# AI-sandbox/gnomix

Measured on AMD Instinct MI355X. Metric: haplotypes/sec (+ windows/sec) chr22 7-ancestry inference, higher is better.
Workload: dtype int8 x 7-digit fixed-point weights -> exact i32/i64 logits, f64 sigmoid (logistic base); f32 (tree smoother)

## Files before the change

gnomix_amd/_lib.py:

```python
from __future__ import annotations

import atexit
import ctypes as C
import os
import weakref

_HERE = os.path.dirname(os.path.abspath(__file__))
SO_PATH = os.environ.get("GNX_LIBRARY") or os.path.join(_HERE, "libgnomix_hip.so")

GNX_ABI_VERSION = 16
GNX_OK, GNX_EINVAL, GNX_ENOMEM, GNX_EHIP, GNX_EUNSUPPORTED, GNX_ESTATE, GNX_ESTALE = 0, -1, -2, -3, -4, -5, -6
BASE_NONE, BASE_LOGISTIC, BASE_COVRSK_SVC, BASE_FOREST, BASE_RFOREST, BASE_KNN, BASE_NB, BASE_LDA = 0, 1, 2, 3, 4, 5, 6, 7
SVC_KERNEL_SUBSTRINGS, SVC_KERNEL_POLY, SVC_KERNEL_ALL_LENGTHS, SVC_KERNEL_RBF = 0, 1, 2, 3
SMOOTH_NONE, SMOOTH_XGB, SMOOTH_CRF, SMOOTH_CNN = 0, 1, 2, 3
K_BASE_LOGISTIC, K_SMOOTH_XGB, K_BASE_COVRSK, K_SMOOTH_CRF, K_GNOFIX, K_SMOOTH_ROWS, K_CALIBRATE, K_BASE_FOREST, K_SMOOTH_CNN = range(9)
KERNEL_NAMES = {K_BASE_LOGISTIC: "k_base_logistic", K_SMOOTH_XGB: "k_smooth_xgb", K_BASE_COVRSK: "k_base_covrsk",
                K_SMOOTH_CRF: "k_smooth_crf", K_GNOFIX: "k_gnofix", K_SMOOTH_ROWS: "k_smooth_rows", K_CALIBRATE: "k_calibrate",
                K_BASE_FOREST: "k_base_forest", K_SMOOTH_CNN: "k_smooth_cnn"}


class GnxLibraryError(ImportError):
    pass


# ... 133 lines not shown
    "gnx_init": (C.c_int, [C.c_int, C.POINTER(_VP)]),
    "gnx_ctx_free": (None, [_VP]),
    "gnx_last_error": (C.c_char_p, [_VP]),
    "gnx_set_stream": (C.c_int, [_VP, _VP]),
    "gnx_reset_stream": (C.c_int, [_VP]),
    "gnx_synchronize": (C.c_int, [_VP]),
    "gnx_model_load": (C.c_int, [_VP, C.POINTER(ModelDesc), C.POINTER(_VP)]),
    "gnx_model_load_nb": (C.c_int, [_VP, C.POINTER(ModelDesc), C.POINTER(NbWindow), C.POINTER(_VP)]),
    "gnx_model_load_lda": (C.c_int, [_VP, C.POINTER(ModelDesc), C.POINTER(LdaWindow), C.POINTER(_VP)]),
    "gnx_model_free": (None, [_VP]),
    "gnx_model_get_info": (C.c_int, [_VP, C.POINTER(ModelInfo)]),
    "gnx_model_set_calibrate": (C.c_int, [_VP, _I]),
    "gnx_model_export_prepared": (C.c_int, [_VP, _VP, _I64, C.POINTER(_I64)]),
    "gnx_base_predict": (C.c_int, [_VP, _VP, _I64, _I64, _VP, _VP]),
    "gnx_base_predict_dev": (C.c_int, [_VP, _VP, _I64, _I64, _VP, _VP]),
    "gnx_smooth_predict": (C.c_int, [_VP, _VP, _I, _I64, _VP, _VP, _VP]),
    "gnx_smooth_predict_dev": (C.c_int, [_VP, _VP, _I, _I64, _VP, _VP, _VP]),
    "gnx_infer": (C.c_int, [_VP, _VP, _I64, _I64, _VP, _VP, _VP]),
    "gnx_infer_dev": (C.c_int, [_VP, _VP, _I64, _I64, _VP, _VP, _VP]),
    "gnx_packed_row_bytes": (_I64, [_I64]),
    "gnx_pack_x": (C.c_int, [_VP, _I64, _I64, _I64, _VP, _I64, _I]),
    "gnx_unpack_x_dev": (C.c_int, [_VP, _VP, _I64, _I64, _I64, _VP, _I64]),
    "gnx_infer_packed": (C.c_int, [_VP, _VP, _I64, _I64, _VP, _VP, _VP]),
    "gnx_infer_packed_dev": (C.c_int, [_VP, _VP, _I64, _I64, _VP, _VP, _VP]),
    "gnx_base_predict_packed_dev": (C.c_int, [_VP, _VP, _I64, _I64, _VP, _VP]),
    "gnx_smooth_rows": (C.c_int, [_VP, _VP, _I64, _VP]),
    "gnx_calibrate_rows": (C.c_int, [_VP, _VP, _I, _I64, _VP]),
    "gnx_gnofix": (C.c_int, [_VP, _VP, _I64, _VP, _I64, C.c_int32, _VP, _VP]),
    "gnx_gnofix_dev": (C.c_int, [_VP, _VP, _I64, _VP, _I64, C.c_int32, _VP, _VP]),
    "gnx_gnofix_packed_dev": (C.c_int, [_VP, _VP, _I64, _VP, _I64, C.c_int32, _VP, _VP]),
# ... 208 lines not shown
```

gnomix_amd/csrc/gnx_api.hip:

```cpp
#include <algorithm>
#include <cmath>
#include <cstdio>
#include <cstdlib>
#include <cstring>
#include <limits>
#include <new>
#include <thread>
#include <utility>

#include "gnx_internal.h"

int gnx_fail(gnx_ctx* ctx, int code, const std::string& msg) {
  if (ctx) ctx->err = msg;
  return code;
}
static inline int fail(gnx_ctx* ctx, int code, const std::string& msg) { return gnx_fail(ctx, code, msg); }

#define HIPCHK(ctx, expr)                                                                      \
  do {                                                                                         \
    hipError_t e__ = (expr);                                                                   \
    if (e__ != hipSuccess)                                                                     \
      return fail((ctx), GNX_EHIP, std::string(#expr) + ": " + hipGetErrorString(e__));        \
  } while (0)

// ... 80 lines not shown
  if (const char* e = std::getenv("GNX_SM_TUNE")) std::sscanf(e, "%d,%d", &t.smf_rpl, &t.smf_nw);
  if (const char* e = std::getenv("GNX_CRF_FLAGS")) t.crf_flags = atoi(e);
  if (const char* e = std::getenv("GNX_LDS_PAD")) std::sscanf(e, "%d,%d", &t.lr_lds_pad, &t.sm_lds_pad);
  if (const char* e = std::getenv("GNX_CRF_IMPL")) t.crf_impl = !std::strcmp(e, "scan") ? 1 : !std::strcmp(e, "row") ? 2 : !std::strcmp(e, "lanes") ? 3 : !std::strcmp(e, "quad") ? 4 : !std::strcmp(e, "mm") ? 5 : 0;
  t.forest_threads = geti("GNX_FOREST_T", 0);
  t.forest_wrun = geti("GNX_FOREST_WRUN", 0);
  t.forest_halves = geti("GNX_FOREST_H", 0);
  t.forest_flags = geti("GNX_FOREST_FLAGS", 0);
  t.forest_impl = geti("GNX_FOREST_IMPL", 0);
  if (const char* e = std::getenv("GNX_HOST_BATCH")) t.host_batch = std::atoll(e);
  t.h2d_overlap = geti("GNX_H2D_OVERLAP", 1);
  t.debug = std::getenv("GNX_DEBUG") ? atoi(std::getenv("GNX_DEBUG")) : 0;
  if (const char* e = std::getenv("GNX_GNOFIX_IMPL")) t.gnofix_impl = std::string(e) == "f32" ? 1 : 0;
  t.gnofix_threads = geti("GNX_GNOFIX_T", 0);
  t.gnofix_aux = geti("GNX_GNOFIX_AUX", 1);
}

extern "C" {

int gnx_abi_version(void) { return GNX_ABI_VERSION; }

int gnx_build_flags(void) {
#ifdef GNX_EXPERIMENTS
  return GNX_BUILD_EXPERIMENTS;
#else
  return 0;
#endif
}

static void want_hw_queues() { setenv("GPU_MAX_HW_QUEUES", "8", 0); }
// ... 270 lines not shown
  if (!m) return;
  gnx_ctx unbound;
  if (!m->ctx) (void)hipGetDevice(&unbound.device);
  gnx_device_scope bind(m->ctx ? m->ctx : &unbound);
  if (m->ctx && m->ctx->usable) (void)hipStreamSynchronize(m->ctx->stream);
  for (void* p : m->dev_allocs) (void)hipFree(p);
  delete m;
}

int gnx_model_get_info(const gnx_model* m, gnx_model_info* out) {
  if (!m || !out) return GNX_EINVAL;
  *out = m->info;
  return GNX_OK;
}

int gnx_base_predict_dev(gnx_model* m, const int8_t* dX, int64_t N, int64_t ldx, float* d_b32, double* d_b64) {
  if (!m) return GNX_EINVAL;
  gnx_ctx* ctx = m->ctx;
  if (N < 0 || ldx < m->info.C || (N > 0 && !dX)) return fail(ctx, GNX_EINVAL, "base_predict: bad X / N / ldx");
  if (N == 0 || (!d_b32 && !d_b64)) return GNX_OK;
  GNX_BIND_DEVICE(ctx);
  if (m->info.base_kind == GNX_BASE_KNN) return gnx_base_predict_knn(m, dX, N, ldx, d_b32, d_b64);
  if (m->info.base_kind == GNX_BASE_NB) return gnx_base_predict_nb(m, dX, N, ldx, d_b32, d_b64);
  if (m->info.base_kind == GNX_BASE_LDA) return gnx_base_predict_lda(m, dX, N, ldx, d_b32, d_b64);
  if (m->info.base_kind == GNX_BASE_COVRSK_SVC && m->rbf) {
    ProfScope ps(ctx, GNX_K_BASE_COVRSK);
    return gnx_base_predict_rbf(m, dX, N, ldx, d_b32, d_b64);
  }
  if (m->info.base_kind == GNX_BASE_COVRSK_SVC) {
    const int64_t Cp = m->info.C + 2 * m->info.ctx, nwp = (Cp + 31) / 32 + 2;
    int rc = ws_reserve(ctx, ctx->ws_bits, (size_t)N * 2 * nwp * 4);
    if (rc != GNX_OK) return rc;
    ProfScope ps(ctx, GNX_K_BASE_COVRSK);
    HIPCHK(ctx, gnx_launch_pack_bits(dX, N, ldx, m->info.C, m->info.ctx, nwp, (uint32_t*)ctx->ws_bits.p, ctx->stream));
    CovRSKLaunch L{};
// ... 48 lines not shown
    const size_t need = (size_t)m->info.C + 128;
    if (ctx->ws_lastrow.cap < need) {
      int rc = ws_reserve(ctx, ctx->ws_lastrow, need);
      if (rc != GNX_OK) return rc;
      HIPCHK(ctx, hipMemsetAsync(ctx->ws_lastrow.p, 0, ctx->ws_lastrow.cap, ctx->stream));
    }
    HIPCHK(ctx, hipMemcpyAsync(ctx->ws_lastrow.p, dX + (N - 1) * ldx, (size_t)m->info.C, hipMemcpyDeviceToDevice, ctx->stream));
  }
  BaseLRLaunch L{};
  L.X = dX;
  L.last_row = (const int8_t*)ctx->ws_lastrow.p;
  L.N = N; L.ldx = ldx; L.d = m->lr;
  L.h_win_chunk0 = m->lr_h_win_chunk0.data(); L.h_win_chunk1 = m->lr_h_win_chunk1.data();
  L.W = (int32_t)m->info.W; L.A = m->info.A;
  L.b32 = d_b32; L.b64 = d_b64;
  ProfScope ps(ctx, GNX_K_BASE_LOGISTIC);
  if (m->lr_i8) {
    const bool dl = ctx->tune.lr_dl < 0 ? m->lr.NT >= 2 : ctx->tune.lr_dl != 0;
    hipError_t e = hipErrorNotSupported;
#ifdef GNX_EXPERIMENTS
    if (ctx->tune.lr_ws) e = gnx_launch_base_logistic_i8_ws(L, ctx->n_cu, ctx->tune, ctx->stream);
    if (e == hipErrorNotSupported && ctx->tune.lr_w512) e = gnx_launch_base_logistic_i8_w512(L, ctx->n_cu, ctx->tune, ctx->stream);
    if (e == hipErrorNotSupported && ctx->tune.lr_flat > 0 && m->lr.V8F) e = gnx_launch_base_logistic_i8_fl(L, ctx->n_cu, ctx->tune, ctx->stream);
#endif
    if (e == hipErrorNotSupported && dl) e = gnx_launch_base_logistic_i8_dl(L, ctx->n_cu, ctx->tune, ctx->stream);
    if (e == hipErrorNotSupported) e = gnx_launch_base_logistic_i8(L, ctx->n_cu, ctx->tune, ctx->stream);
    HIPCHK(ctx, e);
  }
  else HIPCHK(ctx, gnx_launch_base_logistic(L, ctx->n_cu, ctx->stream));
  return GNX_OK;
}

static int smooth_raw_dev(gnx_model* m, const void* dB, int b_is_f64, int64_t N, float* d_p32, double* d_p64, int32_t* d_lab);

int gnx_smooth_predict_dev(gnx_model* m, const void* dB, int b_is_f64, int64_t N, float* d_p32, double* d_p64,
                           int32_t* d_lab) {
  if (!m) return GNX_EINVAL;
  gnx_ctx* ctx = m->ctx;
  GNX_BIND_DEVICE(ctx);
  if (!(m->calibrate_on && m->calib_off)) return smooth_raw_dev(m, dB, b_is_f64, N, d_p32, d_p64, d_lab);
  if (N < 0 || (N > 0 && !dB)) return fail(ctx, GNX_EINVAL, "smooth_predict: bad B / N");
  if (N == 0) return GNX_OK;
  const size_t n = (size_t)N * m->info.W * m->info.A;
  const bool nat64 = m->info.smooth_kind == GNX_SMOOTH_CRF;
  int rc = ws_reserve(ctx, ctx->ws_cal, n * (nat64 ? 8 : 4));
  if (rc != GNX_OK) return rc;
  rc = smooth_raw_dev(m, dB, b_is_f64, N, nat64 ? nullptr : (float*)ctx->ws_cal.p, nat64 ? (double*)ctx->ws_cal.p : nullptr, nullptr);
  if (rc != GNX_OK) return rc;
  CalibLaunch L{};
  L.in = ctx->ws_cal.p; L.in_is_f64 = nat64; L.R = N * m->info.W; L.A = m->info.A;
  L.off = m->calib_off; L.x = m->calib_x; L.y = m->calib_y; L.thr_f32 = m->calib_f32;
  L.out64 = d_p64; L.out32 = d_p32; L.labels = d_lab;
  ProfScope ps(ctx, GNX_K_CALIBRATE);
  HIPCHK(ctx, gnx_launch_calibrate(L, ctx->stream));
  return GNX_OK;
}

static int smooth_raw_dev(gnx_model* m, const void* dB, int b_is_f64, int64_t N, float* d_p32, double* d_p64, int32_t* d_lab) {
  gnx_ctx* ctx = m->ctx;
  if (N < 0 || (N > 0 && !dB)) return fail(ctx, GNX_EINVAL, "smooth_predict: bad B / N");
  if (N == 0) return GNX_OK;
  if (m->info.smooth_kind == GNX_SMOOTH_XGB) {
    const size_t n = (size_t)N * m->info.W * m->info.A;
    if (!d_p32) {
      int rc = ws_reserve(ctx, ctx->ws_misc, n * sizeof(float));
      if (rc != GNX_OK) return rc;
      d_p32 = (float*)ctx->ws_misc.p;
    }
    SmoothXGBLaunch L{};
    L.B = dB; L.b_is_f64 = b_is_f64; L.N = N;
    L.W = (int32_t)m->info.W; L.A = m->info.A; L.S = m->info.S;
    L.d = m->xgb; L.proba = d_p32; L.proba64 = d_p64; L.labels = d_lab;
#ifdef GNX_EXPERIMENTS
    const bool h64 = m->xgb.rk_packed && m->xgb.impl == 2 && gnx_smooth_h64_waves(m->xgb, m->info.A, m->info.S) > 0;
    if (m->xgb.impl == 2 && !h64) return fail(ctx, GNX_EUNSUPPORTED, "GNX_SMOOTH_IMPL=h64: the model's strip does not fit the LDS");
#else
// ... 15 lines not shown
      if (rc != GNX_OK) return rc;
    }
#endif
    ProfScope ps(ctx, GNX_K_SMOOTH_XGB);
#ifdef GNX_EXPERIMENTS
    if (bs) {
      HIPCHK(ctx, gnx_launch_smooth_xgb_bs(L, (uint16_t*)ctx->ws_marg.p, ctx->n_cu, ctx->tune, ctx->stream));
      return GNX_OK;
    }
#endif
#ifdef GNX_EXPERIMENTS
    if (h64) HIPCHK(ctx, gnx_launch_smooth_xgb_h64(L, (uint16_t*)ctx->ws_rank.p, ctx->tune, ctx->stream));
    else
#endif
    if (m->xgb.rk_packed) {
      const bool h32 = (m->xgb.impl == 5 || (m->xgb.impl == 6 && (N + 31) / 32 * ((L.W + GNX_H32_WPB - 1) / GNX_H32_WPB) >= ctx->n_cu)) &&
                       gnx_smooth_h32_fits(m->xgb, L.A, L.S);
      if (h32) {
        HIPCHK(ctx, gnx_launch_smooth_xgb_h32(L, ctx->stream));
        return GNX_OK;
      }
      if (L.d.impl == 5 || L.d.impl == 6) L.d.impl = 3;
      HIPCHK(ctx, gnx_launch_smooth_xgb_rk(L, ctx->tune, ctx->stream));
    } else HIPCHK(ctx, gnx_launch_smooth_xgb(L, ctx->tune, ctx->stream));
    return GNX_OK;
  }
  if (m->info.smooth_kind == GNX_SMOOTH_CRF) {
    const size_t n = (size_t)N * m->info.W * m->info.A;
    int rc;
    if ((rc = ws_reserve(ctx, ctx->ws_misc, n * sizeof(double) + 4096)) != GNX_OK) return rc;
    double* alpha = (double*)ctx->ws_misc.p;
    if ((rc = ws_reserve(ctx, ctx->ws_scale, (size_t)2 * N * m->info.W * sizeof(double))) != GNX_OK) return rc;
    if ((rc = ws_reserve(ctx, ctx->ws_psi, n * sizeof(double) + 4096)) != GNX_OK) return rc;
// ... 57 lines not shown
  const char* in0 = reinterpret_cast<const char*>(dP);
  const bool in_xu = ctx->ws_xu.p && in0 >= (const char*)ctx->ws_xu.p && in0 < (const char*)ctx->ws_xu.p + ctx->ws_xu.cap;
  gnx_devbuf& wide = in_xu ? ctx->ws_xu2 : ctx->ws_xu;
  int rc = ws_reserve(ctx, wide, (size_t)N * ldx + 256);
  if (rc != GNX_OK) return rc;
  HIPCHK(ctx, gnx_launch_unpack2(dP, N, ldp, C, (int8_t*)wide.p, ldx, ctx->stream));
  return gnx_base_predict_dev(m, (const int8_t*)wide.p, N, ldx, d_b32, d_b64);
}

static int infer_any_dev(gnx_model* m, const void* dIn, bool packed, int64_t N, int64_t ld, float* d_p32, double* d_p64, int32_t* d_lab) {
  gnx_ctx* ctx = m->ctx;
  if (N <= 0) return N == 0 ? GNX_OK : fail(ctx, GNX_EINVAL, "infer: N < 0");
  GNX_BIND_DEVICE(ctx);
  const size_t n = (size_t)N * m->info.W * m->info.A;
  const bool f64 = (m->info.smooth_kind == GNX_SMOOTH_CRF);
  int rc = ws_reserve(ctx, f64 ? ctx->ws_b64 : ctx->ws_b32, n * (f64 ? 8 : 4));
  if (rc != GNX_OK) return rc;
  float* b32 = f64 ? nullptr : (float*)ctx->ws_b32.p;
  double* b64 = f64 ? (double*)ctx->ws_b64.p : nullptr;
  rc = packed ? gnx_base_predict_packed_dev(m, (const uint8_t*)dIn, N, ld, b32, b64) : gnx_base_predict_dev(m, (const int8_t*)dIn, N, ld, b32, b64);
  if (rc != GNX_OK) return rc;
  return gnx_smooth_predict_dev(m, f64 ? ctx->ws_b64.p : ctx->ws_b32.p, f64, N, d_p32, d_p64, d_lab);
}

int gnx_infer_dev(gnx_model* m, const int8_t* dX, int64_t N, int64_t ldx, float* d_p32, double* d_p64, int32_t* d_lab) {
  if (!m) return GNX_EINVAL;
  return infer_any_dev(m, dX, false, N, ldx, d_p32, d_p64, d_lab);
}

static int64_t hap_batch(const gnx_model* m, int64_t N, int64_t ldx) {
  int64_t nb = ((int64_t)1 << 30) / std::max<int64_t>(ldx, 1);
// ... 82 lines not shown
  int rc;
  if (nbuf == 2 && (rc = pipe_init(ctx)) != GNX_OK) return rc;
  const int64_t ldx_dev = packed ? ((C + 15) / 16) * 16 : ld;
  const size_t in_bytes = (((size_t)nb * ld + 64) + 255) & ~(size_t)255;
  gnx_devbuf& wsin = packed ? ctx->ws_pk : ctx->ws_x;
  if ((rc = ws_reserve(ctx, wsin, in_bytes * nbuf)) != GNX_OK) return rc;
  const bool p2 = packed && lr_p2_usable(m);
  if (packed && !p2 && (rc = ws_reserve(ctx, ctx->ws_xu, (size_t)nb * ldx_dev + 256)) != GNX_OK) return rc;
  const size_t p32_b = (nb * WA * 4 + 255) & ~(size_t)255, p64_b = (nb * WA * 8 + 255) & ~(size_t)255, lab_b = (nb * Wn * 4 + 255) & ~(size_t)255;
  if ((rc = ws_reserve(ctx, ctx->ws_p32, p32_b * nbuf)) != GNX_OK) return rc;
  if (p64 && (rc = ws_reserve(ctx, ctx->ws_p64, p64_b * nbuf)) != GNX_OK) return rc;
  if (lab && (rc = ws_reserve(ctx, ctx->ws_lab, lab_b * nbuf)) != GNX_OK) return rc;
  {
    const bool f64 = (m->info.smooth_kind == GNX_SMOOTH_CRF);
    if ((rc = ws_reserve(ctx, f64 ? ctx->ws_b64 : ctx->ws_b32, nb * WA * (f64 ? 8 : 4))) != GNX_OK) return rc;
  }
  hipStream_t sc = ctx->stream, si = nbuf == 2 ? ctx->s_in : ctx->stream, so = nbuf == 2 ? ctx->s_out : ctx->stream;
  const uint8_t* hsrc = (const uint8_t*)src;
  const int64_t n_batches = (N + nb - 1) / nb;
  auto issue_h2d = [&](int64_t i) -> int {
    const int b = (int)(i % nbuf);
    const int64_t n0 = i * nb, n = std::min(nb, N - n0);
    if (nbuf == 2 && i >= 2) HIPCHK(ctx, hipStreamWaitEvent(si, ctx->ev_done[b], 0));
    HIPCHK(ctx, hipMemcpyAsync((char*)wsin.p + (size_t)b * in_bytes, hsrc + (size_t)n0 * ld, (size_t)(n - 1) * ld + row_bytes,
                               hipMemcpyHostToDevice, si));
    if (nbuf == 2) HIPCHK(ctx, hipEventRecord(ctx->ev_in[b], si));
    return GNX_OK;
  };
  if ((rc = issue_h2d(0)) != GNX_OK) return rc;
  for (int64_t i = 0; i < n_batches; ++i) {
// ... 681 lines not shown
```

gnomix_amd/csrc/gnx_internal.h:

```cpp
#pragma once
#include <hip/hip_runtime.h>
#include <stdint.h>
#include <algorithm>
#include <memory>
#include <string>
#include <vector>

#include "../../include/gnomix_hip.h"
#include "gnx_rank_table.h"

struct gnx_devbuf {
  void* p = nullptr;
  size_t cap = 0;
};

struct gnx_prof_pair {
  hipEvent_t a, b;
  int kid;
};

struct gnx_tune {
  int lr_bpc = 0, lr_want = 0;
  int lr_mt = 0, lr_waves = 0;
  int lr_flags = 0;
// ... 9 lines not shown
  int sm_pair = 1;
  int smf_rpl = 0, smf_nw = 0;
  int crf_impl = 0;
  int crf_flags = 0;
  int forest_threads = 0;
  int forest_wrun = 0;
  int forest_halves = 0;
  int forest_impl = 0;
  int forest_flags = 0;
  int64_t host_batch = 0;
  int h2d_overlap = 1;
  int lr_lds_pad = 0, sm_lds_pad = 0;
  int gnofix_impl = 0;
  int gnofix_aux = 1;
  int gnofix_threads = 0;
  int debug = 0;
};

#define GNX_LDS_OPTIN(bytes, ...)                                                                                  \
  do {                                                                                                             \
    const hipError_t e_optin_ = hipFuncSetAttribute(reinterpret_cast<const void*>(&__VA_ARGS__),                   \
                                                    hipFuncAttributeMaxDynamicSharedMemorySize, (int)(bytes));     \
    if (e_optin_ != hipSuccess) return e_optin_;                                                                   \
  } while (0)

struct gnx_ctx {
  int device = 0;
  gnx_tune tune;
  hipStream_t stream = nullptr;
  bool own_stream = false;
// ... 51 lines not shown
  const int8_t* X;
  const int8_t* last_row;
  int64_t N, ldx;
  BaseLRDev d;
  const int32_t* h_win_chunk0;
  const int32_t* h_win_chunk1;
  int32_t W, A, wch;
  int32_t n_htiles;
  int32_t n_rg8;
  int32_t flags;
  int32_t max_chunks;
  int32_t max_wins;
  float* b32;
  double* b64;
  unsigned long long* dbg = nullptr;
};

struct SmoothXGBDev {
  const uint8_t* packed = nullptr;
  const int32_t* group_tree0 = nullptr;
  const int32_t* group_class = nullptr;
  int32_t n_groups = 0, n_trees = 0, D = 0, tree_bytes = 0, max_group = 0;
  float base_score = 0.5f;
  const uint8_t* rk_packed = nullptr;
  const float* rk_thr = nullptr;
  const GnxRankEntry* rk_lut = nullptr;
  const int32_t* rk_group_tree0 = nullptr;
  const int32_t* rk_group_class = nullptr;
  int32_t rk_K = 0, rk_steps = 0, rk_stride = 0, rk_tree_bytes = 0, rk_n_groups = 0, rk_max_group = 0;
  int32_t rk_bits = 0;
  int32_t rk_rpl = 0;
// ... 61 lines not shown
  __builtin_memcpy(&fv, row + n4.x, 4);
  return (fv < __uint_as_float(n4.y)) ? __uint_as_float(n4.z) : __uint_as_float(n4.w);
}
#endif

struct SmoothXGBLaunch {
  const void* B;
  int32_t b_is_f64;
  int64_t N;
  int32_t W, A, S;
  SmoothXGBDev d;
  float* proba;
  float* marg;
  double* proba64;
  int32_t* labels;
};


struct SmoothCRFLaunch {
  const void* B;
  int32_t b_is_f64;
  int64_t N;
  int32_t W, A;
  const double* state;
  const double* etrans;
  double* psi;
  double* alpha;
  double* scale;
  double* proba64;
  float* proba32;
// ... 219 lines not shown
  *out = (const T*)p;
  return GNX_OK;
}


hipError_t gnx_launch_gt2_to_x(const uint8_t* G, int64_t V, int64_t ldg, int64_t n0, int64_t N, const int32_t* src, int64_t C,
                               int8_t* X, int64_t ldx, hipStream_t s);
hipError_t gnx_launch_gt2_to_p2(const uint8_t* G, int64_t V, int64_t ldg, int64_t n0, int64_t N, const int32_t* src, int64_t C,
                                uint8_t* P, int64_t ldp, hipStream_t s);
hipError_t gnx_launch_p2_to_gt2(const uint8_t* P, int64_t N, int64_t ldp, int64_t n0, const int32_t* cols, int64_t V, uint8_t* G,
                                int64_t ldg, hipStream_t s);
hipError_t gnx_launch_x_to_gt2(const int8_t* X, int64_t N, int64_t ldx, int64_t n0, const int32_t* cols, int64_t V, uint8_t* G,
                               int64_t ldg, hipStream_t s);
hipError_t gnx_launch_base_logistic(const BaseLRLaunch& L, int n_cu, hipStream_t s);
hipError_t gnx_launch_base_logistic_i8(const BaseLRLaunch& L, int n_cu, const gnx_tune& tune, hipStream_t s);
hipError_t gnx_launch_base_logistic_i8_dl(const BaseLRLaunch& L, int n_cu, const gnx_tune& tune, hipStream_t s);
hipError_t gnx_launch_base_logistic_p2(const BaseLRLaunch& L, int n_cu, const gnx_tune& tune, hipStream_t s);
#ifdef GNX_EXPERIMENTS
hipError_t gnx_launch_base_logistic_i8_w512(const BaseLRLaunch& L, int n_cu, const gnx_tune& tune, hipStream_t s);
hipError_t gnx_launch_base_logistic_i8_ws(const BaseLRLaunch& L, int n_cu, const gnx_tune& tune, hipStream_t s);
hipError_t gnx_launch_base_logistic_i8_fl(const BaseLRLaunch& L, int n_cu, const gnx_tune& tune, hipStream_t s);
hipError_t gnx_launch_smooth_xgb_h64(const SmoothXGBLaunch& L, uint16_t* Rk, const gnx_tune& tune, hipStream_t s);
int gnx_smooth_h64_waves(const SmoothXGBDev& d, int A, int S);
size_t gnx_smooth_h64_rank_bytes(int64_t N, int W, int A, int S);
#endif
hipError_t gnx_launch_fb_len(const float* d_proba, int64_t N, int64_t W, int A, uint8_t* d_len, unsigned long long* d_line_len, hipStream_t s);
hipError_t gnx_launch_fb_emit(const float* d_proba, int64_t N, int64_t W, int A, const uint8_t* d_len, const char* d_pb, const int64_t* d_po,
                              const int64_t* d_line_off, char* d_body, hipStream_t s);
hipError_t gnx_launch_smooth_xgb(const SmoothXGBLaunch& L, const gnx_tune& tune, hipStream_t s);
hipError_t gnx_launch_smooth_xgb_rk(const SmoothXGBLaunch& L, const gnx_tune& tune, hipStream_t s);
// ... 45 lines not shown
```

gnomix_amd/csrc/k_base_logistic_i8.hip:

```cpp
#include <algorithm>
#include <cstdio>
#include <cstdlib>

#include "gnx_internal.h"
#include "gnx_exp.h"

namespace {

typedef int v4i __attribute__((ext_vector_type(4)));
struct __attribute__((packed, aligned(1))) xbytes16 { v4i v; };

constexpr int LIMBS = 7;

__device__ __forceinline__ v4i load_x16(const int8_t* p) {
  xbytes16 r;
  __builtin_memcpy(&r, p, 16);
  return r.v;
}

__device__ __forceinline__ double combine(const v4i (&acc)[LIMBS], int reg, double scale) {
  long long lo = (long long)acc[0][reg] + ((long long)acc[1][reg] << 8) + ((long long)acc[2][reg] << 16);
  long long hi = (long long)acc[3][reg] + ((long long)acc[4][reg] << 8) + ((long long)acc[5][reg] << 16) +
                 ((long long)acc[6][reg] << 24);
  return ((double)hi * 16777216.0 + (double)lo) * scale;
// ... 18 lines not shown
    const int last_ = min(CPS, c_end - c0_) * (CHUNK_BYTES / 16) - 1;                                 \
    const v4i* src_ = reinterpret_cast<const v4i*>(L.d.V8 + (size_t)c0_ * CHUNK_BYTES);           \
    _Pragma("unroll") for (int v = 0; v < VPT; ++v) VS[v] = src_[min(v * THREADS + tid, last_)];      \
  }

#define GNX_STAGE_STORE(XS, VS, STEP)                                                                 \
  {                                                                                                   \
    _Pragma("unroll") for (int q = 0; q < XPT; ++q) *reinterpret_cast<v4i*>(xt + fslot[q]) = XS[q];   \
    v4i* dst_ = reinterpret_cast<v4i*>(vbuf + (size_t)((STEP) & 1) * STEP_BYTES);                 \
    _Pragma("unroll") for (int v = 0; v < VPT; ++v) {                                                 \
      const int e_ = v * THREADS + tid;                                                               \
      if (e_ < STEP_BYTES / 16) dst_[e_] = VS[v];                                                     \
    }                                                                                                 \
  }

template <int MT, int NT, int WAVES, int CPS>
__global__ __launch_bounds__(WAVES * 64) void k_base_logistic_i8(BaseLRLaunch L) {
  static_assert(CPS == 2, "a step is 2 chunks = 8 pieces of 16 SNPs");
  extern __shared__ __attribute__((aligned(16))) uint8_t lds[];
  constexpr int CHUNK_BYTES = NT * LIMBS * 1024;
  constexpr int STEP_BYTES = CPS * CHUNK_BYTES;
  constexpr int THREADS = WAVES * 64;
  constexpr int ROWS = WAVES * MT * 16;
  constexpr int XT_BYTES = ROWS * 128;
  constexpr int XPT = ROWS * 8 / THREADS;
  constexpr int VPT = (STEP_BYTES / 16 + THREADS - 1) / THREADS;
  const int tid = threadIdx.x, lane = tid & 63, wave = tid >> 6;
  const int i16 = lane & 15, kq = lane >> 4;
  const int A = L.A, W = L.W, R = L.d.R;
  uint8_t* xt = lds;
  uint8_t* vbuf = lds + XT_BYTES;
// ... 109 lines not shown
            double* z = zb + lane * A;
            double sum = 0.0;
            for (int a = 0; a < A; ++a) {
              const double p = gnx_sigmoid(z[a] + tab_ic[(w - wt0) * A + a]);
              z[a] = p;
              sum += p;
            }
            if (n < L.N) {
              const size_t o = ((size_t)n * W + w) * A;
              const double rs = gnx_rcp_nr(sum);
              for (int a = 0; a < A; ++a) {
                const double v = z[a] * rs;
                if (L.b64) L.b64[o + a] = v;
                if (L.b32) L.b32[o + a] = (float)v;
              }
            }
          }
          asm volatile("s_waitcnt lgkmcnt(0)" ::: "memory");
        }
      }
    }
  };

  GNX_STAGE_LOAD(xsA, vsA, 0);
  GNX_STAGE_STORE(xsA, vsA, 0);
  GNX_STAGE_LOAD(xsB, vsB, 1);
  __syncthreads();

  for (int s = 0; s < n_steps; s += 2) {
    GNX_STAGE_LOAD(xsA, vsA, s + 2);
    compute_step(s);
    GNX_LDS_BARRIER();
    GNX_STAGE_STORE(xsB, vsB, s + 1);
    GNX_LDS_BARRIER();
    GNX_STAGE_LOAD(xsB, vsB, s + 3);
    compute_step(s + 1);
    GNX_LDS_BARRIER();
    GNX_STAGE_STORE(xsA, vsA, s + 2);
    GNX_LDS_BARRIER();
  }
}
#undef GNX_LDS_BARRIER
#undef GNX_STAGE_LOAD
#undef GNX_STAGE_STORE

template <int MT, int NT, int WAVES, int CPS>
hipError_t launch(const BaseLRLaunch& L, int n_cu, const gnx_tune& tune, hipStream_t s) {
  BaseLRLaunch P = L;
  const int haps_per_block = WAVES * MT * 16;
  const int64_t gx = (L.N + haps_per_block - 1) / haps_per_block;
  const int bpc = tune.lr_bpc > 0 ? tune.lr_bpc : 4;
  int64_t want = ((int64_t)bpc * n_cu + gx - 1) / gx;
  want = std::max<int64_t>(8, ((want + 7) / 8) * 8);
  if (tune.lr_want > 0) want = tune.lr_want;
  int wch = 0, n_ranges = 0;
  size_t lds = 0;
  for (;; want += 8) {
    wch = (int)((L.W + want - 1) / want);
    if (wch < 4) wch = 4;
    n_ranges = (L.W + wch - 1) / wch;
    int max_chunks = 0;
// ... 5 lines not shown
      max_chunks += 8;
    } else {
      max_chunks = (wch + L.d.R + 2) * L.d.max_piece_chunks + 8;
    }
    P.max_chunks = max_chunks;
    P.max_wins = wch + 2 * L.d.R + 4;
    lds = (size_t)WAVES * MT * 16 * 128 + (size_t)2 * CPS * NT * LIMBS * 1024 + (size_t)WAVES * MT * 16 * L.A * sizeof(double) +
          (size_t)3 * P.max_chunks * sizeof(int) + (size_t)P.max_wins * (L.A + 1) * sizeof(double);
    if (lds <= (size_t)160 * 1024 || wch == 4) break;
  }
  if (lds > (size_t)160 * 1024) return hipErrorInvalidValue;
  lds = std::min(lds + (size_t)std::max(tune.lr_lds_pad, 0), (size_t)160 * 1024);
  const int n_ranges8 = ((n_ranges + 7) / 8) * 8;
  P.wch = wch;
  P.n_htiles = (int)gx;
  GNX_LDS_OPTIN(lds, k_base_logistic_i8<MT, NT, WAVES, CPS>);
  hipLaunchKernelGGL((k_base_logistic_i8<MT, NT, WAVES, CPS>), dim3((unsigned)(gx * n_ranges8)), dim3(WAVES * 64), lds, s, P);
  const hipError_t e = hipGetLastError();
  if (e != hipSuccess && tune.debug) std::fprintf(stderr, "k_base_logistic_i8<%d,%d,%d>: lds=%zu grid=%lld wch=%d max_chunks=%d max_wins=%d\n", MT, NT, WAVES, lds, (long long)(gx * n_ranges8), wch, P.max_chunks, P.max_wins);
  return e;
}

}

hipError_t gnx_launch_base_logistic_i8(const BaseLRLaunch& L0, int n_cu, const gnx_tune& tune, hipStream_t s) {
  if (L0.N <= 0) return hipSuccess;
  BaseLRLaunch L = L0;
  const bool small = L.N <= 64 * 8;
  const int tm = tune.lr_mt, tw = tune.lr_waves;
  L.flags = tune.lr_flags;
  if (L.d.NT == 1 && tm) {
    if (tm == 1 && tw == 4) return launch<1, 1, 4, 2>(L, n_cu, tune, s);
    if (tm == 1 && tw == 8) return launch<1, 1, 8, 2>(L, n_cu, tune, s);
    if (tm == 1 && tw == 16) return launch<1, 1, 16, 2>(L, n_cu, tune, s);
    if (tm == 2 && tw == 4) return launch<2, 1, 4, 2>(L, n_cu, tune, s);
    if (tm == 2 && tw == 8) return launch<2, 1, 8, 2>(L, n_cu, tune, s);
    if (tm == 4 && tw == 4) return launch<4, 1, 4, 2>(L, n_cu, tune, s);
    if (tm == 4 && tw == 8) return launch<4, 1, 8, 2>(L, n_cu, tune, s);
    return hipErrorInvalidValue;
  }
  if (L.d.NT == 2 && tm) {
    if (tm == 1 && tw == 4) return launch<1, 2, 4, 2>(L, n_cu, tune, s);
    if (tm == 1 && tw == 8) return launch<1, 2, 8, 2>(L, n_cu, tune, s);
// ... 14 lines not shown
```

gnomix_amd/csrc/k_smooth_xgb_h32.hip:

```cpp
#include <cstdio>
#include <cstdlib>

#include "gnx_internal.h"
#include "gnx_exp.h"
#include "gnx_rank.h"

namespace {

constexpr int HB = 32;
constexpr int RW = 3;
constexpr int NWAVE = 16;
constexpr int WPW = 2 * RW;
constexpr int WPB = NWAVE * WPW;
constexpr int THREADS = NWAVE * 64;
constexpr int TB = GNX_H32_TREE_BYTES;
static_assert(WPB == GNX_H32_WPB, "the model loader sizes the staging groups for this block");

#if defined(__HIP_DEVICE_COMPILE__)
template <typename T>
__device__ __forceinline__ const __attribute__((address_space(3))) T* lds_at(uint32_t a) {
  return (const __attribute__((address_space(3))) T*)(uintptr_t)a;
}
#else
template <typename T>
// ... 47 lines not shown
    }
#pragma unroll
    for (int c = 0; c < NC; ++c) r[c] = *lds_at<uint16_t>(rb[c % RW] + (w0[c] & 0xffffu));
#pragma unroll
    for (int c = 0; c < NC; ++c) p[c] = step_ptr(w0[c], w1[c], r[c]);
  }
  float lf[NC];
#pragma unroll
  for (int c = 0; c < NC; ++c) lf[c] = *lds_at<float>(p[c]);
#pragma unroll
  for (int t = 0; t < NT; ++t)
#pragma unroll
    for (int k = 0; k < RW; ++k) psum[k] += lf[t * RW + k];
}

__global__ __launch_bounds__(THREADS, 8) void k_smooth_xgb_h32(SmoothXGBLaunch L, int gw) {
  extern __shared__ __attribute__((aligned(16))) uint8_t lds[];
  const int A = L.A, W = L.W, S = L.S, pad = (S + 1) / 2;
  const int buf_bytes = L.d.h3_max_group * TB;
  const int P = WPB + S - 1;
  uint8_t* tbuf0 = lds;
  uint8_t* tbuf1 = tbuf0 + buf_bytes;
  uint8_t* strip = tbuf1 + buf_bytes;
  const int tid = threadIdx.x, lane = tid & 63, wave = tid >> 6, h = lane & 31, hv = lane >> 5;
  const int64_t hb = blockIdx.y, h0 = hb * HB;
  const int w0 = blockIdx.x * WPB;

  {
    constexpr int NV = 4;
    const int per_h = P * A;
    const int hl = (wave & 1) * 16 + (lane >> 2);
    const size_t row = (size_t)min(h0 + hl, L.N - 1) * W;
    const int dq = 32 / A, da = 32 - dq * A;
    int rr = (wave >> 1) * 4 + (lane & 3);
    int q = rr / A, a = rr - q * A;
    const bool interior = w0 >= pad && w0 + P <= pad + W;
    const size_t run0 = (row + (size_t)(interior ? w0 - pad : 0)) * A;
    for (; rr < per_h; rr += NV * 32) {
      float p[NV];
      uint32_t r[NV];
      int dst[NV];
      bool ok[NV];
      if (interior) {
// ... 152 lines not shown

}

bool gnx_smooth_h32_fits(const SmoothXGBDev& d, int A, int S) {
  return d.h3_packed && d.rk_thr && d.D == 4 && lds_need(d, A, S) <= (size_t)80 * 1024;
}

hipError_t gnx_launch_smooth_xgb_h32(const SmoothXGBLaunch& L, hipStream_t s) {
  if (L.N <= 0) return hipSuccess;
  if (!gnx_smooth_h32_fits(L.d, L.A, L.S)) return hipErrorInvalidValue;
  const size_t lds = lds_need(L.d, L.A, L.S);
  int gw = NWAVE;
  while (gw > 1 && (size_t)HB * ((size_t)(gw * WPW * L.A) | 1) * 4 > lds) gw >>= 1;
  if ((size_t)HB * ((size_t)(gw * WPW * L.A) | 1) * 4 > lds) return hipErrorInvalidValue;
  const dim3 grid((unsigned)((L.W + WPB - 1) / WPB), (unsigned)((L.N + HB - 1) / HB));
  GNX_LDS_OPTIN(lds, k_smooth_xgb_h32);
  hipLaunchKernelGGL(k_smooth_xgb_h32, grid, dim3(THREADS), lds, s, L, gw);
  return hipGetLastError();
}
```

include/gnomix_hip.h:

```cpp
#ifndef GNOMIX_HIP_H
#define GNOMIX_HIP_H

#include <stddef.h>
#include <stdint.h>

#ifdef __cplusplus
extern "C" {
#endif

#define GNX_ABI_VERSION 16

typedef struct gnx_ctx gnx_ctx;
typedef struct gnx_model gnx_model;

enum {
  GNX_OK = 0,
  GNX_EINVAL = -1,
  GNX_ENOMEM = -2,
  GNX_EHIP = -3,
  GNX_EUNSUPPORTED = -4,
  GNX_ESTATE = -5,
  GNX_ESTALE = -6
};

// ... 151 lines not shown
int gnx_host_free(gnx_ctx* ctx, void* p);
#define GNX_HOST_PORTABLE 0x1u
int gnx_host_flags(const void* p, unsigned* flags);
int gnx_debug_ws_devices(gnx_ctx* ctx, int32_t* out, int32_t n);

int gnx_model_load(gnx_ctx* ctx, const gnx_model_desc* desc, gnx_model** out);
int gnx_model_load_nb(gnx_ctx* ctx, const gnx_model_desc* desc, const gnx_nb_window* nb , gnx_model** out);
int gnx_model_load_lda(gnx_ctx* ctx, const gnx_model_desc* desc, const gnx_lda_window* lda , gnx_model** out);
void gnx_model_free(gnx_model* model);
int gnx_model_get_info(const gnx_model* model, gnx_model_info* out);
int gnx_model_set_calibrate(gnx_model* model, int on);
int gnx_model_export_prepared(gnx_model* model, void* buf, int64_t cap, int64_t* bytes);

int gnx_base_predict(gnx_model* model, const int8_t* X, int64_t N, int64_t ldx, float* b_f32, double* b_f64);
int gnx_base_predict_dev(gnx_model* model, const int8_t* dX, int64_t N, int64_t ldx, float* d_b_f32, double* d_b_f64);

int gnx_smooth_predict(gnx_model* model, const void* B, int b_is_f64, int64_t N, float* proba_f32,
                       double* proba_f64, int32_t* labels);
int gnx_smooth_predict_dev(gnx_model* model, const void* dB, int b_is_f64, int64_t N, float* d_proba_f32,
                           double* d_proba_f64, int32_t* d_labels);

int gnx_infer(gnx_model* model, const int8_t* X, int64_t N, int64_t ldx, float* proba_f32, double* proba_f64,
              int32_t* labels);
int gnx_infer_dev(gnx_model* model, const int8_t* dX, int64_t N, int64_t ldx, float* d_proba_f32,
                  double* d_proba_f64, int32_t* d_labels);

int64_t gnx_packed_row_bytes(int64_t C);
int gnx_pack_x(const int8_t* X, int64_t N, int64_t ldx, int64_t C, uint8_t* packed, int64_t ldp, int n_threads);
int gnx_unpack_x_dev(gnx_ctx* ctx, const uint8_t* d_packed, int64_t N, int64_t ldp, int64_t C, int8_t* dX, int64_t ldx);
int gnx_infer_packed(gnx_model* model, const uint8_t* packed, int64_t N, int64_t ldp, float* proba_f32, double* proba_f64,
// ... 193 lines not shown
```

Before: 3.751 million.

## Emit smoother rank image from base logistic kernel and feed it to h32 smoother

Result: faster. 3.872 million, median of 6 (+3.2%).

```diff
diff --git a/gnomix_amd/_lib.py b/gnomix_amd/_lib.py
--- a/gnomix_amd/_lib.py
+++ b/gnomix_amd/_lib.py
@@ -171,6 +171,7 @@
     "gnx_model_export_prepared": (C.c_int, [_VP, _VP, _I64, C.POINTER(_I64)]),
     "gnx_base_predict": (C.c_int, [_VP, _VP, _I64, _I64, _VP, _VP]),
     "gnx_base_predict_dev": (C.c_int, [_VP, _VP, _I64, _I64, _VP, _VP]),
+    "gnx_base_predict_ranks_dev": (C.c_int, [_VP, _VP, _I64, _I64, _VP, _VP]),
     "gnx_smooth_predict": (C.c_int, [_VP, _VP, _I, _I64, _VP, _VP, _VP]),
     "gnx_smooth_predict_dev": (C.c_int, [_VP, _VP, _I, _I64, _VP, _VP, _VP]),
     "gnx_infer": (C.c_int, [_VP, _VP, _I64, _I64, _VP, _VP, _VP]),
diff --git a/gnomix_amd/csrc/gnx_api.hip b/gnomix_amd/csrc/gnx_api.hip
--- a/gnomix_amd/csrc/gnx_api.hip
+++ b/gnomix_amd/csrc/gnx_api.hip
@@ -118,6 +118,7 @@
   if (const char* e = std::getenv("GNX_GNOFIX_IMPL")) t.gnofix_impl = std::string(e) == "f32" ? 1 : 0;
   t.gnofix_threads = geti("GNX_GNOFIX_T", 0);
   t.gnofix_aux = geti("GNX_GNOFIX_AUX", 1);
+  t.fuse_ranks = geti("GNX_FUSE_RANKS", 1);
 }
 
 extern "C" {
@@ -418,11 +419,35 @@
   return GNX_OK;
 }
 
+static bool base_can_rank(const gnx_model* m) {
+  const gnx_tune& t = m->ctx->tune;
+  if (m->info.base_kind != GNX_BASE_LOGISTIC || !m->lr_i8 || !m->xgb.rk_thr || !m->xgb.rk_lut) return false;
+#ifdef GNX_EXPERIMENTS
+  if (t.lr_ws || t.lr_w512 || (t.lr_flat > 0 && m->lr.V8F)) return false;
+#endif
+  const bool dl = t.lr_dl < 0 ? m->lr.NT >= 2 : t.lr_dl != 0;
+  return !dl && gnx_base_logistic_i8_ranks(m->lr, t);
+}
+
+static int base_predict_dev(gnx_model* m, const int8_t* dX, int64_t N, int64_t ldx, float* d_b32, double* d_b64, uint16_t* d_rk16);
+
 int gnx_base_predict_dev(gnx_model* m, const int8_t* dX, int64_t N, int64_t ldx, float* d_b32, double* d_b64) {
+  return base_predict_dev(m, dX, N, ldx, d_b32, d_b64, nullptr);
+}
+
+int gnx_base_predict_ranks_dev(gnx_model* m, const int8_t* dX, int64_t N, int64_t ldx, float* d_b32, uint16_t* d_rk16) {
+  if (!m) return GNX_EINVAL;
+  if (!d_rk16) return fail(m->ctx, GNX_EINVAL, "base_predict_ranks: no rank image");
+  if (!base_can_rank(m)) return fail(m->ctx, GNX_EUNSUPPORTED, "base_predict_ranks: this model's base pass does not write ranks");
+  return base_predict_dev(m, dX, N, ldx, d_b32, nullptr, d_rk16);
+}
+
+static int base_predict_dev(gnx_model* m, const int8_t* dX, int64_t N, int64_t ldx, float* d_b32, double* d_b64, uint16_t* d_rk16) {
   if (!m) return GNX_EINVAL;
   gnx_ctx* ctx = m->ctx;
   if (N < 0 || ldx < m->info.C || (N > 0 && !dX)) return fail(ctx, GNX_EINVAL, "base_predict: bad X / N / ldx");
-  if (N == 0 || (!d_b32 && !d_b64)) return GNX_OK;
+  if (N == 0 || (!d_b32 && !d_b64 && !d_rk16)) return GNX_OK;
+  if (d_rk16 && !base_can_rank(m)) return fail(ctx, GNX_ESTATE, "base_predict: a rank image from a base pass that writes none");
   GNX_BIND_DEVICE(ctx);
   if (m->info.base_kind == GNX_BASE_KNN) return gnx_base_predict_knn(m, dX, N, ldx, d_b32, d_b64);
   if (m->info.base_kind == GNX_BASE_NB) return gnx_base_predict_nb(m, dX, N, ldx, d_b32, d_b64);
@@ -501,6 +526,11 @@
   L.h_win_chunk0 = m->lr_h_win_chunk0.data(); L.h_win_chunk1 = m->lr_h_win_chunk1.data();
   L.W = (int32_t)m->info.W; L.A = m->info.A;
   L.b32 = d_b32; L.b64 = d_b64;
+  if (d_rk16) {
+    L.rk16 = d_rk16;
+    L.rk_thr = m->xgb.rk_thr; L.rk_lut = m->xgb.rk_lut;
+    L.rk_K = m->xgb.rk_K; L.rk_bits = m->xgb.rk_bits; L.rk_steps = m->xgb.rk_steps;
+  }
   ProfScope ps(ctx, GNX_K_BASE_LOGISTIC);
   if (m->lr_i8) {
     const bool dl = ctx->tune.lr_dl < 0 ? m->lr.NT >= 2 : ctx->tune.lr_dl != 0;
@@ -518,21 +548,35 @@
   return GNX_OK;
 }
 
-static int smooth_raw_dev(gnx_model* m, const void* dB, int b_is_f64, int64_t N, float* d_p32, double* d_p64, int32_t* d_lab);
+static int smooth_raw_dev(gnx_model* m, const void* dB, int b_is_f64, int64_t N, float* d_p32, double* d_p64, int32_t* d_lab,
+                          const uint16_t* d_rk16 = nullptr);
+static int smooth_predict_dev(gnx_model* m, const void* dB, int b_is_f64, int64_t N, float* d_p32, double* d_p64, int32_t* d_lab,
+                              const uint16_t* d_rk16);
 
 int gnx_smooth_predict_dev(gnx_model* m, const void* dB, int b_is_f64, int64_t N, float* d_p32, double* d_p64,
                            int32_t* d_lab) {
-  if (!m) return GNX_EINVAL;
-  gnx_ctx* ctx = m->ctx;
-  GNX_BIND_DEVICE(ctx);
-  if (!(m->calibrate_on && m->calib_off)) return smooth_raw_dev(m, dB, b_is_f64, N, d_p32, d_p64, d_lab);
-  if (N < 0 || (N > 0 && !dB)) return fail(ctx, GNX_EINVAL, "smooth_predict: bad B / N");
+  return smooth_predict_dev(m, dB, b_is_f64, N, d_p32, d_p64, d_lab, nullptr);
+}
+
+static bool smooth_takes_h32(const gnx_model* m, int64_t N) {
+  if (m->info.smooth_kind != GNX_SMOOTH_XGB || !m->xgb.rk_packed) return false;
+  const int64_t blocks = (N + 31) / 32 * ((m->info.W + GNX_H32_WPB - 1) / GNX_H32_WPB);
+  return (m->xgb.impl == 5 || (m->xgb.impl == 6 && blocks >= m->ctx->n_cu)) && gnx_smooth_h32_fits(m->xgb, m->info.A, m->info.S);
+}
+
+static int smooth_predict_dev(gnx_model* m, const void* dB, int b_is_f64, int64_t N, float* d_p32, double* d_p64, int32_t* d_lab,
+                              const uint16_t* d_rk16) {
+  if (!m) return GNX_EINVAL;
+  gnx_ctx* ctx = m->ctx;
+  GNX_BIND_DEVICE(ctx);
+  if (!(m->calibrate_on && m->calib_off)) return smooth_raw_dev(m, dB, b_is_f64, N, d_p32, d_p64, d_lab, d_rk16);
+  if (N < 0 || (N > 0 && !dB && !d_rk16)) return fail(ctx, GNX_EINVAL, "smooth_predict: bad B / N");
   if (N == 0) return GNX_OK;
   const size_t n = (size_t)N * m->info.W * m->info.A;
   const bool nat64 = m->info.smooth_kind == GNX_SMOOTH_CRF;
   int rc = ws_reserve(ctx, ctx->ws_cal, n * (nat64 ? 8 : 4));
   if (rc != GNX_OK) return rc;
-  rc = smooth_raw_dev(m, dB, b_is_f64, N, nat64 ? nullptr : (float*)ctx->ws_cal.p, nat64 ? (double*)ctx->ws_cal.p : nullptr, nullptr);
+  rc = smooth_raw_dev(m, dB, b_is_f64, N, nat64 ? nullptr : (float*)ctx->ws_cal.p, nat64 ? (double*)ctx->ws_cal.p : nullptr, nullptr, d_rk16);
   if (rc != GNX_OK) return rc;
   CalibLaunch L{};
   L.in = ctx->ws_cal.p; L.in_is_f64 = nat64; L.R = N * m->info.W; L.A = m->info.A;
@@ -543,10 +587,12 @@
   return GNX_OK;
 }
 
-static int smooth_raw_dev(gnx_model* m, const void* dB, int b_is_f64, int64_t N, float* d_p32, double* d_p64, int32_t* d_lab) {
-  gnx_ctx* ctx = m->ctx;
-  if (N < 0 || (N > 0 && !dB)) return fail(ctx, GNX_EINVAL, "smooth_predict: bad B / N");
+static int smooth_raw_dev(gnx_model* m, const void* dB, int b_is_f64, int64_t N, float* d_p32, double* d_p64, int32_t* d_lab,
+                          const uint16_t* d_rk16) {
+  gnx_ctx* ctx = m->ctx;
+  if (N < 0 || (N > 0 && !dB && !d_rk16)) return fail(ctx, GNX_EINVAL, "smooth_predict: bad B / N");
   if (N == 0) return GNX_OK;
+  if (d_rk16 && !smooth_takes_h32(m, N)) return fail(ctx, GNX_ESTATE, "smooth_predict: a rank image for a smoother that reads none");
   if (m->info.smooth_kind == GNX_SMOOTH_XGB) {
     const size_t n = (size_t)N * m->info.W * m->info.A;
     if (!d_p32) {
@@ -592,9 +638,8 @@
     else
 #endif
     if (m->xgb.rk_packed) {
-      const bool h32 = (m->xgb.impl == 5 || (m->xgb.impl == 6 && (N + 31) / 32 * ((L.W + GNX_H32_WPB - 1) / GNX_H32_WPB) >= ctx->n_cu)) &&
-                       gnx_smooth_h32_fits(m->xgb, L.A, L.S);
-      if (h32) {
+      if (smooth_takes_h32(m, N)) {
+        L.rk16 = d_rk16;
         HIPCHK(ctx, gnx_launch_smooth_xgb_h32(L, ctx->stream));
         return GNX_OK;
       }
@@ -682,7 +727,20 @@
   GNX_BIND_DEVICE(ctx);
   const size_t n = (size_t)N * m->info.W * m->info.A;
   const bool f64 = (m->info.smooth_kind == GNX_SMOOTH_CRF);
-  int rc = ws_reserve(ctx, f64 ? ctx->ws_b64 : ctx->ws_b32, n * (f64 ? 8 : 4));
+  int rc;
+  if (!packed && ctx->tune.fuse_ranks != 0 && base_can_rank(m) && smooth_takes_h32(m, N)) {
+    if ((rc = ws_reserve(ctx, ctx->ws_rank, gnx_rank_image_bytes(N, (int)m->info.W, m->info.A))) != GNX_OK) return rc;
+    uint16_t* rk16 = (uint16_t*)ctx->ws_rank.p;
+#ifdef GNX_FUSE_ABLATE
+    if ((rc = ws_reserve(ctx, ctx->ws_b32, n * 4)) != GNX_OK) return rc;
+    if ((rc = base_predict_dev(m, (const int8_t*)dIn, N, ld, (float*)ctx->ws_b32.p, nullptr, GNX_FUSE_ABLATE == 2 ? rk16 : nullptr)) != GNX_OK) return rc;
+    return smooth_predict_dev(m, ctx->ws_b32.p, 0, N, d_p32, d_p64, d_lab, GNX_FUSE_ABLATE == 1 ? rk16 : nullptr);
+#else
+    if ((rc = base_predict_dev(m, (const int8_t*)dIn, N, ld, nullptr, nullptr, rk16)) != GNX_OK) return rc;
+    return smooth_predict_dev(m, nullptr, 0, N, d_p32, d_p64, d_lab, rk16);
+#endif
+  }
+  rc = ws_reserve(ctx, f64 ? ctx->ws_b64 : ctx->ws_b32, n * (f64 ? 8 : 4));
   if (rc != GNX_OK) return rc;
   float* b32 = f64 ? nullptr : (float*)ctx->ws_b32.p;
   double* b64 = f64 ? (double*)ctx->ws_b64.p : nullptr;
@@ -795,6 +853,8 @@
   {
     const bool f64 = (m->info.smooth_kind == GNX_SMOOTH_CRF);
     if ((rc = ws_reserve(ctx, f64 ? ctx->ws_b64 : ctx->ws_b32, nb * WA * (f64 ? 8 : 4))) != GNX_OK) return rc;
+    if (!packed && ctx->tune.fuse_ranks != 0 && base_can_rank(m) && m->info.smooth_kind == GNX_SMOOTH_XGB &&
+        (rc = ws_reserve(ctx, ctx->ws_rank, gnx_rank_image_bytes(nb, (int)m->info.W, m->info.A))) != GNX_OK) return rc;
   }
   hipStream_t sc = ctx->stream, si = nbuf == 2 ? ctx->s_in : ctx->stream, so = nbuf == 2 ? ctx->s_out : ctx->stream;
   const uint8_t* hsrc = (const uint8_t*)src;
diff --git a/gnomix_amd/csrc/gnx_internal.h b/gnomix_amd/csrc/gnx_internal.h
--- a/gnomix_amd/csrc/gnx_internal.h
+++ b/gnomix_amd/csrc/gnx_internal.h
@@ -47,6 +47,7 @@
   int gnofix_impl = 0;
   int gnofix_aux = 1;
   int gnofix_threads = 0;
+  int fuse_ranks = 1;
   int debug = 0;
 };
 
@@ -128,7 +129,12 @@
   float* b32;
   double* b64;
   unsigned long long* dbg = nullptr;
-};
+  uint16_t* rk16 = nullptr;
+  const float* rk_thr = nullptr;
+  const GnxRankEntry* rk_lut = nullptr;
+  int32_t rk_K = 0, rk_bits = 0, rk_steps = 0;
+};
+inline size_t gnx_rank_image_bytes(int64_t N, int W, int A) { return (size_t)((N + 31) / 32) * 32 * (size_t)W * (size_t)A * sizeof(uint16_t); }
 
 struct SmoothXGBDev {
   const uint8_t* packed = nullptr;
@@ -220,6 +226,7 @@
   float* marg;
   double* proba64;
   int32_t* labels;
+  const uint16_t* rk16 = nullptr;
 };
 
 
@@ -469,6 +476,7 @@
                                int64_t ldg, hipStream_t s);
 hipError_t gnx_launch_base_logistic(const BaseLRLaunch& L, int n_cu, hipStream_t s);
 hipError_t gnx_launch_base_logistic_i8(const BaseLRLaunch& L, int n_cu, const gnx_tune& tune, hipStream_t s);
+bool gnx_base_logistic_i8_ranks(const BaseLRDev& d, const gnx_tune& tune);
 hipError_t gnx_launch_base_logistic_i8_dl(const BaseLRLaunch& L, int n_cu, const gnx_tune& tune, hipStream_t s);
 hipError_t gnx_launch_base_logistic_p2(const BaseLRLaunch& L, int n_cu, const gnx_tune& tune, hipStream_t s);
 #ifdef GNX_EXPERIMENTS
diff --git a/gnomix_amd/csrc/k_base_logistic_i8.hip b/gnomix_amd/csrc/k_base_logistic_i8.hip
--- a/gnomix_amd/csrc/k_base_logistic_i8.hip
+++ b/gnomix_amd/csrc/k_base_logistic_i8.hip
@@ -4,6 +4,7 @@
 
 #include "gnx_internal.h"
 #include "gnx_exp.h"
+#include "gnx_rank.h"
 
 namespace {
 
@@ -56,7 +57,7 @@
     }                                                                                                 \
   }
 
-template <int MT, int NT, int WAVES, int CPS>
+template <int MT, int NT, int WAVES, int CPS, bool RK = false>
 __global__ __launch_bounds__(WAVES * 64) void k_base_logistic_i8(BaseLRLaunch L) {
   static_assert(CPS == 2, "a step is 2 chunks = 8 pieces of 16 SNPs");
   extern __shared__ __attribute__((aligned(16))) uint8_t lds[];
@@ -196,6 +197,20 @@
                 if (L.b64) L.b64[o + a] = v;
                 if (L.b32) L.b32[o + a] = (float)v;
               }
+              if constexpr (RK) {
+                constexpr int RNV = 4;
+                uint16_t* rrow = L.rk16 + (((size_t)(n >> 5) * W + w) * A) * 32 + (n & 31);
+                for (int a0 = 0; a0 < A; a0 += RNV) {
+                  float pf[RNV];
+                  uint32_t rr[RNV];
+#pragma unroll
+                  for (int i = 0; i < RNV; ++i) pf[i] = (float)(z[min(a0 + i, A - 1)] * rs);
+                  ranks<RNV>(L.rk_thr, L.rk_lut, L.rk_K, L.rk_bits, L.rk_steps, pf, rr);
+#pragma unroll
+                  for (int i = 0; i < RNV; ++i)
+                    if (a0 + i < A) rrow[(size_t)(a0 + i) * 32] = (uint16_t)rr[i];
+                }
+              }
             }
           }
           asm volatile("s_waitcnt lgkmcnt(0)" ::: "memory");
@@ -226,7 +241,7 @@
 #undef GNX_STAGE_LOAD
 #undef GNX_STAGE_STORE
 
-template <int MT, int NT, int WAVES, int CPS>
+template <int MT, int NT, int WAVES, int CPS, bool RK = false>
 hipError_t launch(const BaseLRLaunch& L, int n_cu, const gnx_tune& tune, hipStream_t s) {
   BaseLRLaunch P = L;
   const int haps_per_block = WAVES * MT * 16;
@@ -262,19 +277,26 @@
   const int n_ranges8 = ((n_ranges + 7) / 8) * 8;
   P.wch = wch;
   P.n_htiles = (int)gx;
-  GNX_LDS_OPTIN(lds, k_base_logistic_i8<MT, NT, WAVES, CPS>);
-  hipLaunchKernelGGL((k_base_logistic_i8<MT, NT, WAVES, CPS>), dim3((unsigned)(gx * n_ranges8)), dim3(WAVES * 64), lds, s, P);
+  GNX_LDS_OPTIN(lds, k_base_logistic_i8<MT, NT, WAVES, CPS, RK>);
+  hipLaunchKernelGGL((k_base_logistic_i8<MT, NT, WAVES, CPS, RK>), dim3((unsigned)(gx * n_ranges8)), dim3(WAVES * 64), lds, s, P);
   const hipError_t e = hipGetLastError();
   if (e != hipSuccess && tune.debug) std::fprintf(stderr, "k_base_logistic_i8<%d,%d,%d>: lds=%zu grid=%lld wch=%d max_chunks=%d max_wins=%d\n", MT, NT, WAVES, lds, (long long)(gx * n_ranges8), wch, P.max_chunks, P.max_wins);
   return e;
 }
 
 }
+
+bool gnx_base_logistic_i8_ranks(const BaseLRDev& d, const gnx_tune& tune) { return d.NT == 1 && tune.lr_mt == 0; }
 
 hipError_t gnx_launch_base_logistic_i8(const BaseLRLaunch& L0, int n_cu, const gnx_tune& tune, hipStream_t s) {
   if (L0.N <= 0) return hipSuccess;
   BaseLRLaunch L = L0;
   const bool small = L.N <= 64 * 8;
+  if (L.rk16) {
+    if (!gnx_base_logistic_i8_ranks(L.d, tune) || !L.rk_thr || !L.rk_lut) return hipErrorInvalidValue;
+    L.flags = tune.lr_flags;
+    return small ? launch<1, 1, 4, 2, true>(L, n_cu, tune, s) : launch<2, 1, 8, 2, true>(L, n_cu, tune, s);
+  }
   const int tm = tune.lr_mt, tw = tune.lr_waves;
   L.flags = tune.lr_flags;
   if (L.d.NT == 1 && tm) {
diff --git a/gnomix_amd/csrc/k_smooth_xgb_h32.hip b/gnomix_amd/csrc/k_smooth_xgb_h32.hip
--- a/gnomix_amd/csrc/k_smooth_xgb_h32.hip
+++ b/gnomix_amd/csrc/k_smooth_xgb_h32.hip
@@ -85,6 +85,7 @@
     for (int k = 0; k < RW; ++k) psum[k] += lf[t * RW + k];
 }
 
+template <bool IMG>
 __global__ __launch_bounds__(THREADS, 8) void k_smooth_xgb_h32(SmoothXGBLaunch L, int gw) {
   extern __shared__ __attribute__((aligned(16))) uint8_t lds[];
   const int A = L.A, W = L.W, S = L.S, pad = (S + 1) / 2;
@@ -97,7 +98,39 @@
   const int64_t hb = blockIdx.y, h0 = hb * HB;
   const int w0 = blockIdx.x * WPB;
 
-  {
+  if constexpr (IMG) {
+    constexpr int RPI = THREADS / 4;
+    const int n_rows = ((P + 1) / 2) * A;
+    const uint16_t* img = L.rk16 + (size_t)hb * W * A * HB + (tid & 3) * 8;
+    const int dq = RPI / A, da = RPI - dq * A;
+    int row = tid >> 2;
+    int q = row / A, a = row - q * A;
+    for (int it = 0; it < (n_rows + RPI - 1) / RPI; ++it, row += RPI) {
+      const bool ok = row < n_rows;
+      const int qc = ok ? q : 0, ac = ok ? a : 0;
+      const int s0 = slide_src(min(w0 + 2 * qc, W + 2 * pad - 1), W, pad);
+      const int s1 = slide_src(min(w0 + 2 * qc + 1, W + 2 * pad - 1), W, pad);
+      const u32x4 x = *reinterpret_cast<const u32x4*>(img + ((size_t)s0 * A + ac) * HB);
+      const u32x4 y = *reinterpret_cast<const u32x4*>(img + ((size_t)s1 * A + ac) * HB);
+      u32x4 lo4, hi4;
+      lo4.x = (x.x & 0xffffu) | (y.x << 16);
+      lo4.y = (x.x >> 16) | (y.x & 0xffff0000u);
+      lo4.z = (x.y & 0xffffu) | (y.y << 16);
+      lo4.w = (x.y >> 16) | (y.y & 0xffff0000u);
+      hi4.x = (x.z & 0xffffu) | (y.z << 16);
+      hi4.y = (x.z >> 16) | (y.z & 0xffff0000u);
+      hi4.z = (x.w & 0xffffu) | (y.w << 16);
+      hi4.w = (x.w >> 16) | (y.w & 0xffff0000u);
+      if (ok) {
+        u32x4* dst = reinterpret_cast<u32x4*>(strip + (size_t)row * 128 + (tid & 3) * 32);
+        dst[0] = lo4;
+        dst[1] = hi4;
+      }
+      a += da;
+      q += dq;
+      if (a >= A) { a -= A; ++q; }
+    }
+  } else {
     constexpr int NV = 4;
     const int per_h = P * A;
     const int hl = (wave & 1) * 16 + (lane >> 2);
@@ -280,7 +313,12 @@
   while (gw > 1 && (size_t)HB * ((size_t)(gw * WPW * L.A) | 1) * 4 > lds) gw >>= 1;
   if ((size_t)HB * ((size_t)(gw * WPW * L.A) | 1) * 4 > lds) return hipErrorInvalidValue;
   const dim3 grid((unsigned)((L.W + WPB - 1) / WPB), (unsigned)((L.N + HB - 1) / HB));
-  GNX_LDS_OPTIN(lds, k_smooth_xgb_h32);
-  hipLaunchKernelGGL(k_smooth_xgb_h32, grid, dim3(THREADS), lds, s, L, gw);
+  if (L.rk16) {
+    GNX_LDS_OPTIN(lds, k_smooth_xgb_h32<true>);
+    hipLaunchKernelGGL(k_smooth_xgb_h32<true>, grid, dim3(THREADS), lds, s, L, gw);
+  } else {
+    GNX_LDS_OPTIN(lds, k_smooth_xgb_h32<false>);
+    hipLaunchKernelGGL(k_smooth_xgb_h32<false>, grid, dim3(THREADS), lds, s, L, gw);
+  }
   return hipGetLastError();
 }
diff --git a/include/gnomix_hip.h b/include/gnomix_hip.h
--- a/include/gnomix_hip.h
+++ b/include/gnomix_hip.h
@@ -189,6 +189,7 @@
 
 int gnx_base_predict(gnx_model* model, const int8_t* X, int64_t N, int64_t ldx, float* b_f32, double* b_f64);
 int gnx_base_predict_dev(gnx_model* model, const int8_t* dX, int64_t N, int64_t ldx, float* d_b_f32, double* d_b_f64);
+int gnx_base_predict_ranks_dev(gnx_model* model, const int8_t* dX, int64_t N, int64_t ldx, float* d_b_f32, uint16_t* d_rk16);
 
 int gnx_smooth_predict(gnx_model* model, const void* B, int b_is_f64, int64_t N, float* proba_f32,
                        double* proba_f64, int32_t* labels);
```
